# aouyang1/go-muse

Hardware: AMD Instinct MI355X
Metric: series-pairs XCorr/sec at N=4096, 1M-series batch; achieved HBM GB/s (higher is better)
Workload: dtype f64

## Files before the change

### go-muse_amd/csrc/foldk_device.h

```cpp
#pragma once
#include <hip/hip_runtime.h>
#include <stdint.h>

#include "fold_device.h"
#include "r16_device.h"

namespace muse {

namespace foldk {

using namespace occ4;
using namespace fold;

constexpr int XW = 544;

template <int PERM>
__device__ __forceinline__ constexpr int pr(int k)
{
    return PERM ? BR16(k) : k;
}

template <int MODE, int PERM, bool TAILBAR = false>
__device__ __forceinline__ void exchange_cross(double2 (&v)[16], double2 *xbuf, const int wave, const int t_, const int wcol = -1)
{
// ... 60 lines not shown
    const int rbase = 272 * hl + 17 * lo;
#pragma unroll
    for (int k = 0; k < 16; k++)
        lds_st2(xw + 17 * k + wbase, v[pr<PERM>(k)]);
    fence();
    asm volatile("" ::: "memory");
    fence();
#pragma unroll
    for (int e = 0; e < 16; e++)
        v[e] = lds_ld2(xw + rbase + e);
}

#if defined(__HIP_DEVICE_COMPILE__)
typedef __attribute__((address_space(3))) char *lds_ptr;
#define MUSE_LDS_ADDR(p) ((unsigned)(unsigned long long)(lds_ptr)(p))
#else
#define MUSE_LDS_ADDR(p) 0u
#endif
template <int PERM>
__device__ __forceinline__ void exchange_local(double2 (&v)[16], double2 *xw, const int t_)
{
    const int t = t_;
    const int hl = (t >> 4) & 3, lo = t & 15;
    const int wbase = 17 * hl + lo;
    const int rbase = 68 * (lo & 7) + 17 * hl;
#pragma unroll
    for (int k = 0; k < 8; k++)
        lds_st2(xw + 68 * k + wbase, v[pr<PERM>(k)]);
    const unsigned waddr = MUSE_LDS_ADDR(xw + wbase), raddr = MUSE_LDS_ADDR(xw + rbase);
    const unsigned long long first = __ballot(lo < 8);
    d2v w[16], d[8];
#pragma unroll
    for (int k = 0; k < 8; k++) {
        d[k].x = v[pr<PERM>(8 + k)].x;
        d[k].y = v[pr<PERM>(8 + k)].y;
    }
    unsigned long long sv;
    asm volatile("s_mov_b64 %[sv], exec\n\t"
                 "s_and_b64 exec, %[sv], %[m]\n\t"
                 "ds_read_b128 %[w0], %[ra]\n\t"
                 "ds_read_b128 %[w1], %[ra] offset:16\n\t"
                 "ds_read_b128 %[w2], %[ra] offset:32\n\t"
                 "ds_read_b128 %[w3], %[ra] offset:48\n\t"
                 "ds_read_b128 %[w4], %[ra] offset:64\n\t"
                 "ds_read_b128 %[w5], %[ra] offset:80\n\t"
                 "ds_read_b128 %[w6], %[ra] offset:96\n\t"
                 "ds_read_b128 %[w7], %[ra] offset:112\n\t"
                 "ds_read_b128 %[w8], %[ra] offset:128\n\t"
                 "ds_read_b128 %[w9], %[ra] offset:144\n\t"
                 "ds_read_b128 %[w10], %[ra] offset:160\n\t"
                 "ds_read_b128 %[w11], %[ra] offset:176\n\t"
                 "ds_read_b128 %[w12], %[ra] offset:192\n\t"
                 "ds_read_b128 %[w13], %[ra] offset:208\n\t"
                 "ds_read_b128 %[w14], %[ra] offset:224\n\t"
                 "ds_read_b128 %[w15], %[ra] offset:240\n\t"
                 "s_mov_b64 exec, %[sv]\n\t"
                 "ds_write_b128 %[wa], %[d0]\n\t"
                 "ds_write_b128 %[wa], %[d1] offset:1088\n\t"
                 "ds_write_b128 %[wa], %[d2] offset:2176\n\t"
                 "ds_write_b128 %[wa], %[d3] offset:3264\n\t"
                 "ds_write_b128 %[wa], %[d4] offset:4352\n\t"
                 "ds_write_b128 %[wa], %[d5] offset:5440\n\t"
                 "ds_write_b128 %[wa], %[d6] offset:6528\n\t"
                 "ds_write_b128 %[wa], %[d7] offset:7616\n\t"
                 "s_andn2_b64 exec, %[sv], %[m]\n\t"
                 "ds_read_b128 %[w0], %[ra]\n\t"
                 "ds_read_b128 %[w1], %[ra] offset:16\n\t"
                 "ds_read_b128 %[w2], %[ra] offset:32\n\t"
                 "ds_read_b128 %[w3], %[ra] offset:48\n\t"
                 "ds_read_b128 %[w4], %[ra] offset:64\n\t"
                 "ds_read_b128 %[w5], %[ra] offset:80\n\t"
                 "ds_read_b128 %[w6], %[ra] offset:96\n\t"
                 "ds_read_b128 %[w7], %[ra] offset:112\n\t"
                 "ds_read_b128 %[w8], %[ra] offset:128\n\t"
                 "ds_read_b128 %[w9], %[ra] offset:144\n\t"
                 "ds_read_b128 %[w10], %[ra] offset:160\n\t"
                 "ds_read_b128 %[w11], %[ra] offset:176\n\t"
                 "ds_read_b128 %[w12], %[ra] offset:192\n\t"
                 "ds_read_b128 %[w13], %[ra] offset:208\n\t"
                 "ds_read_b128 %[w14], %[ra] offset:224\n\t"
                 "ds_read_b128 %[w15], %[ra] offset:240\n\t"
                 "s_mov_b64 exec, %[sv]\n\t"
                 "s_waitcnt lgkmcnt(0)"
                 : [w0] "=&v"(w[0]), [w1] "=&v"(w[1]), [w2] "=&v"(w[2]), [w3] "=&v"(w[3]), [w4] "=&v"(w[4]),
                   [w5] "=&v"(w[5]), [w6] "=&v"(w[6]), [w7] "=&v"(w[7]), [w8] "=&v"(w[8]), [w9] "=&v"(w[9]),
                   [w10] "=&v"(w[10]), [w11] "=&v"(w[11]), [w12] "=&v"(w[12]), [w13] "=&v"(w[13]),
                   [w14] "=&v"(w[14]), [w15] "=&v"(w[15]), [sv] "=&s"(sv)
                 : [ra] "v"(raddr), [wa] "v"(waddr), [m] "s"(first), [d0] "v"(d[0]), [d1] "v"(d[1]), [d2] "v"(d[2]),
                   [d3] "v"(d[3]), [d4] "v"(d[4]), [d5] "v"(d[5]), [d6] "v"(d[6]), [d7] "v"(d[7])
                 : "memory", "scc");
#pragma unroll
    for (int e = 0; e < 16; e++)
        v[e] = make_double2(w[e].x, w[e].y);
}

struct G2Fetch {
    const double2 *p;
    int j;
    __device__ __forceinline__ double2 operator()(int s) const { return p[16 * s + j]; }
};
struct G3Fetch {
    const double2 *p;
    int t;
    __device__ __forceinline__ double2 operator()(int s) const
    {
        return ldg2(scalar_ptr_at(p, ((s + 1) & ~1) * 256), t - 256 * (s & 1));
    }
};

struct G3Derived {
    double2 g[8];
    __device__ __forceinline__ static double2 sq(const double2 w) { return make_double2(fma_(w.x, w.x, -(w.y * w.y)), (w.x + w.x) * w.y); }
    __device__ __forceinline__ static double2 mulc(const double2 w, const double c, const double s)
    {
        return make_double2(fma_(w.y, s, w.x * c), fma_(-w.x, s, w.y * c));
    }
    __device__ __forceinline__ G3Derived(const double2 *tab, int t)
    {
        constexpr double H = 0.70710678118654752440;
        const double2 w8 = G3Fetch{tab, t}(2), w16 = G3Fetch{tab, t}(4);
        g[2] = w8;
        g[4] = w16;
        g[1] = sq(w8);
        g[0] = sq(g[1]);
        g[3] = make_double2(H * (w8.x + w8.y), H * (w8.y - w8.x));
        g[5] = mulc(w16, C16_1, S16_1);
        g[6] = make_double2(H * (w16.x + w16.y), H * (w16.y - w16.x));
        g[7] = mulc(w16, S16_1, C16_1);
    }
    __device__ __forceinline__ double2 operator()(int s) const { return g[s]; }
};

template <typename F>
__device__ __forceinline__ void gdft16_nr_l2(double2 (&v)[16], F fetch)
{
    double2 ga[4], gb[4];
#pragma unroll
    for (int s = 0; s < 4; s++)
        ga[s] = fetch(s);
    gdft16_nr_s12(v, ga[0], ga[1]);
    fence();
#pragma unroll
    for (int s = 0; s < 4; s++)
        gb[s] = fetch(4 + s);
    fence();
    gdft16_nr_s3(v, ga[2], ga[3]);
    fence();
    fence();
    gdft16_nr_s4(v, gb[0], gb[1], gb[2], gb[3]);
}

constexpr int REC = 36;

__device__ __forceinline__ bool finalize(const double *r, const int series, const double invN, const double invNm1,
                                         double *mv_out, int *lag_out)
{
    double m[4], s[4], ix[4];
#pragma unroll
    for (int w = 0; w < 4; w++) {
        m[w] = r[6 * w + 3 * series];
        s[w] = r[6 * w + 3 * series + 1];
        ix[w] = r[6 * w + 3 * series + 2];
    }
    const double s2 = (r[24 + series] + r[26 + series]) + (r[28 + series] + r[30 + series]);
    const Stat st{r[32 + series], s2};
    double best = m[0], bsv = s[0], bidx = ix[0];
#pragma unroll
    for (int w = 1; w < 4; w++) {
        if (m[w] > best || (m[w] == best && ix[w] < bidx)) {
            best = m[w];
            bsv = s[w];
            bidx = ix[w];
        }
    }
    bool zero, nan;
    const double var = variance(st, invN, invNm1, zero, nan);
    const int idx = (best > 0.0) ? (int)bidx : 0;
    double y = __builtin_amdgcn_rsq(var);
    y = y * fma(-0.5 * var * y, y, 1.5);
    y = y * fma(-0.5 * var * y, y, 1.5);
    double mv = ((best > 0.0) ? bsv : s[0]) * y;
    int lag = idx > 2048 ? idx - 4096 : idx;
    if (zero) { mv = 0.0; lag = 0; }
    if (nan) { mv = __builtin_nan(""); lag = 0; }
    *mv_out = mv;
    *lag_out = lag;
    bool redo = nan;
    if (series == 0 && r[35] != 0.0) {
        const double s2b = (r[25] + r[27]) + (r[29] + r[31]);
        const Stat sb{r[33], s2b};
        bool zb, nb;
        const double varb = variance(sb, invN, invNm1, zb, nb);
        redo = redo || (!nb && sigma_spread_too_wide(var, varb));
    }
    return redo;
}

#define MUSE_HIWORD_CASE(m) case m: h = __builtin_amdgcn_readlane(__double2hiint(S == 0 ? v[BR16(m)].x : v[BR16(m)].y), l); break;
template <int S>
__device__ __forceinline__ int hiword_at(const double2 (&v)[16], const int m, const int l)
{
    int h = 0;
    switch (m) {
        MUSE_HIWORD_CASE(0) MUSE_HIWORD_CASE(1) MUSE_HIWORD_CASE(2) MUSE_HIWORD_CASE(3)
        MUSE_HIWORD_CASE(4) MUSE_HIWORD_CASE(5) MUSE_HIWORD_CASE(6) MUSE_HIWORD_CASE(7)
        MUSE_HIWORD_CASE(8) MUSE_HIWORD_CASE(9) MUSE_HIWORD_CASE(10) MUSE_HIWORD_CASE(11)
        MUSE_HIWORD_CASE(12) MUSE_HIWORD_CASE(13) MUSE_HIWORD_CASE(14) MUSE_HIWORD_CASE(15)
    }
    return h;
}
#undef MUSE_HIWORD_CASE
__device__ __forceinline__ void lowest_hit(const unsigned acc, int &m_out, int &l_out)
{
    unsigned long long c = __ballot(acc != 0u);
    int bm = 16, bl = 0;
    while (c != 0ull) {
        const int l = __ffsll((long long)c) - 1;
        const int m = __ffs((int)__builtin_amdgcn_readlane((int)acc, l)) - 1;
        if (m < bm) {
            bm = m;
            bl = l;
        }
        c &= c - 1ull;
    }
    m_out = bm;
    l_out = bl;
}
__device__ __forceinline__ void wave_argmax_store(const double2 (&v)[16], const int wave, const int lane, double *ra_)
{
    double ma = 0.0, mb = 0.0;
#pragma unroll
    for (int k = 0; k < 16; k++) {
        ma = fmax(ma, fabs(v[k].x));
        mb = fmax(mb, fabs(v[k].y));
    }
    const double wa = wave_max_nonneg(ma), wb = wave_max_nonneg(mb);
    unsigned accA = 0u, accB = 0u;
#pragma unroll
    for (int m = 15; m >= 0; m--) {
        const int k = BR16(m);
        asm("v_cmp_eq_f64 vcc, |%1|, %2\n\tv_addc_co_u32 %0, vcc, %0, %0, vcc" : "+v"(accA) : "v"(v[k].x), "s"(wa) : "vcc");
        asm("v_cmp_eq_f64 vcc, |%1|, %2\n\tv_addc_co_u32 %0, vcc, %0, %0, vcc" : "+v"(accB) : "v"(v[k].y), "s"(wb) : "vcc");
    }
    int widxA = 0x7fffffff, widxB = 0x7fffffff;
    double svA = 0.0, svB = 0.0;
    if (__double_as_longlong(wa) != 0ll) {
        int m, l;
        lowest_hit(accA, m, l);
        if (m < 16) {
            widxA = wave * 64 + l + 256 * m;
            svA = (hiword_at<0>(v, m, l) < 0) ? -wa : wa;
        }
    }
    if (__double_as_longlong(wb) != 0ll) {
        int m, l;
        lowest_hit(accB, m, l);
        if (m < 16) {
            widxB = wave * 64 + l + 256 * m;
            svB = (hiword_at<1>(v, m, l) < 0) ? -wb : wb;
        }
    }
    const double cc0a = v[0].x, cc0b = v[0].y;
    if (lane == 0) {
        ra_[0] = widxA == 0x7fffffff ? 0.0 : wa;
        ra_[1] = widxA == 0x7fffffff ? cc0a : svA;
        ra_[2] = (double)widxA;
        ra_[3] = widxB == 0x7fffffff ? 0.0 : wb;
        ra_[4] = widxB == 0x7fffffff ? cc0b : svB;
        ra_[5] = (double)widxB;
    }
}

template <int S>
__device__ __forceinline__ void wave_argmax_store_one(const double2 (&v)[16], const int wave, const int lane, double *out3)
{
    double ma = 0.0;
#pragma unroll
    for (int k = 0; k < 16; k++)
        ma = fmax(ma, fabs(S == 0 ? v[k].x : v[k].y));
    const double wa = wave_max_nonneg(ma);
    unsigned acc = 0u;
#pragma unroll
    for (int m = 15; m >= 0; m--) {
        const int k = BR16(m);
        asm("v_cmp_eq_f64 vcc, |%1|, %2\n\tv_addc_co_u32 %0, vcc, %0, %0, vcc" : "+v"(acc) : "v"(S == 0 ? v[k].x : v[k].y), "s"(wa) : "vcc");
    }
    int widx = 0x7fffffff;
    double sv = 0.0;
    if (__double_as_longlong(wa) != 0ll) {
        int m, l;
        lowest_hit(acc, m, l);
        if (m < 16) {
            widx = wave * 64 + l + 256 * m;
            sv = (hiword_at<S>(v, m, l) < 0) ? -wa : wa;
        }
    }
    const double cc0 = S == 0 ? v[0].x : v[0].y;
    if (lane == 0) {
        out3[0] = widx == 0x7fffffff ? 0.0 : wa;
        out3[1] = widx == 0x7fffffff ? cc0 : sv;
        out3[2] = (double)widx;
    }
}

__device__ __forceinline__ void xc_stage1_pre(double2 (&v)[16], const double2 (&xf)[16])
{
#pragma unroll
    for (int i = 0; i < 4; i++) {
        bf_xc(v[BR16(2 * i)], v[BR16(2 * i) + 1], xf[2 * i], xf[2 * i + 8]);
        bf_xc(v[BR16(2 * i + 1)], v[BR16(2 * i + 1) + 1], xf[2 * i + 1], xf[2 * i + 9]);
    }
}

template <typename F>
__device__ __forceinline__ void xc_stage1(double2 (&v)[16], F xcl)
{
    double2 xa[4], xb[4];
#define MUSE_XC_LOAD(dst, i)          \
    dst[0] = xcl(2 * (i));            \
    dst[1] = xcl(2 * (i) + 8);        \
    dst[2] = xcl(2 * (i) + 1);        \
    dst[3] = xcl(2 * (i) + 9);
#define MUSE_XC_USE(src, i)                                                      \
    bf_xc(v[BR16(2 * (i))], v[BR16(2 * (i)) + 1], src[0], src[1]);               \
    bf_xc(v[BR16(2 * (i) + 1)], v[BR16(2 * (i) + 1) + 1], src[2], src[3]);
    MUSE_XC_LOAD(xa, 0)
    MUSE_XC_LOAD(xb, 1)
    fence();
    MUSE_XC_USE(xa, 0)
    fence();
    MUSE_XC_LOAD(xa, 2)
    MUSE_XC_USE(xb, 1)
    fence();
    MUSE_XC_LOAD(xb, 3)
    MUSE_XC_USE(xa, 2)
    fence();
    MUSE_XC_USE(xb, 3)
#undef MUSE_XC_LOAD
#undef MUSE_XC_USE
}

}

}
```

### go-muse_amd/csrc/n4096_pair_device.h

```cpp
#pragma once
#include "foldk_device.h"

namespace muse {

namespace foldk {

#if defined(__HIP_DEVICE_COMPILE__)
typedef d2v __attribute__((address_space(1))) *zc_out_ptr;
typedef double __attribute__((address_space(1))) *zstat_out_ptr;
typedef const double __attribute__((address_space(4))) *zstat_in_ptr;
#endif

struct PairThread {
    int t, lane, wave;
    double invN, invNm1;
};
template <bool PADDED>
__device__ __forceinline__ PairThread pair_prologue(const FusedParams &p, double2 *g2s, double *prev_row, const int rec_stride)
{
    PairThread th;
    th.t = threadIdx.x;
    th.lane = th.t & 63;
    th.wave = __builtin_amdgcn_readfirstlane(th.t >> 6);
    th.invN = PADDED ? p.invN : 1.0 / 4096.0;
    th.invNm1 = PADDED ? p.invNm1 : 1.0 / 4095.0;
    if (th.t < 128)
        g2s[th.t] = p.g2[th.t];
    if (th.t < 2)
        prev_row[rec_stride * th.t] = -1.0;
    return th;
}

template <bool PIN>
__device__ __forceinline__ int tl(const int t)
{
    int x = t;
    if (PIN)
        asm volatile("" : "+v"(x));
    return x;
}

template <typename T>
__device__ __forceinline__ gptr<T> lane_entry(const T *tab, const long long off, const int j, const int t)
{
    return scalar_ptr_at(tab, off + 256 * ((j + 1) & ~1)) + (t - 256 * (j & 1));
}
struct XcFetch {
    const double2 *xcp;
    int t;
    __device__ __forceinline__ double2 operator()(int j) const { return ldg2(lane_entry(xcp, 0, j, t), 0); }
};

template <bool PADDED, bool F32, bool SLIDE = false>
__device__ __forceinline__ void request_rows(RawPair &raw, const FusedParams &p, const long long pr, const int t, const int pad)
{
    constexpr bool WIDE = !PADDED && !F32;
    if (SLIDE && WIDE)
        issue_row_loads_wide_slide(raw, p, pr, t);
    else if (SLIDE && F32)
        issue_row_loads_slide<PADDED>(raw, p.rows32, p, pr, t, pad);
    else if (SLIDE)
        issue_row_loads_slide<PADDED>(raw, p.rows, p, pr, t, pad);
    else if (WIDE)
        issue_row_loads_wide(raw, p, pr, t);
    else
        issue_row_loads<PADDED, F32>(raw, p, pr, t, pad);
}

#define MUSE_CONSUME_ROWS(WIDE, raw, v, part, t, lane, wave, rA, hasB)      \
    {                                                                       \
        const double KA = (raw).ka, KB = (raw).kb;                          \
        double qa = 0.0, qb = 0.0;                                          \
        if (WIDE)                                                           \
            widen_rows(raw);                                                \
        _Pragma("unroll") for (int i = 0; i < 16; i++) {                    \
            const double da = (raw).a[i] - KA, db = (raw).b[i] - KB;        \
            (v)[i] = make_double2(da, db);                                  \
            qa = fma(da, da, qa);                                           \
            qb = fma(db, db, qb);                                           \
        }                                                                   \
        qa = wave_sum_dpp(qa);                                              \
        qb = wave_sum_dpp(qb);                                              \
        if ((lane) == 0) {                                                  \
            (part)[2 * (wave)] = qa;                                        \
            (part)[2 * (wave) + 1] = qb;                                    \
        }                                                                   \
        if ((t) == 0) {                                                     \
            (part)[10] = (double)(rA);                                      \
            (part)[11] = (hasB) ? 1.0 : 0.0;                                \
        }                                                                   \
    }

template <bool PADDED>
__device__ __forceinline__ void take_dc(double2 (&v)[16], const int t, double &s1a, double &s1b)
{
    s1a = readlane_f64(v[0].x, 0);
    s1b = readlane_f64(v[0].y, 0);
    if (!PADDED) {
        v[0].x = (t == 0) ? 0.0 : v[0].x;
        v[0].y = (t == 0) ? 0.0 : v[0].y;
    }
}

__device__ __forceinline__ void finalize_pair(const double *prec, const int series, const bool writer, const double invN,
                                              const double invNm1, const FusedParams &p)
{
    if (writer && series < 2 && prec[34] >= 0.0 && (series == 0 || prec[35] != 0.0)) {
        const long long row = (long long)prec[34] + series;
        if (finalize(prec, series, invN, invNm1, p.mv + row, p.lag + row)) {
            const int slot = atomicAdd(p.ovf_count, 1);
            p.ovf_list[slot] = row >> 1;
        }
    }
}

struct Nothing {
    __device__ __forceinline__ void operator()() const {}
};
template <int B, typename Between = Nothing>
__device__ __forceinline__ void correct_padded(double2 (&v)[16], const double *c1, const int t, const double mA, const double mB,
                                               Between between = Between())
{
#pragma unroll
    for (int h = 0; h < 16 / B; h++) {
        double cq[B];
#pragma unroll
        for (int k = 0; k < B; k++)
            cq[k] = *lane_entry(c1, 0, B * h + k, t);
        fence();
        between();
#pragma unroll
        for (int k = 0; k < B; k++) {
            const int r = BR16(B * h + k);
            v[r] = make_double2(fma(-mA, cq[k], v[r].x), fma(-mB, cq[k], v[r].y));
        }
    }
}

__device__ __forceinline__ void request_z(d2v (&zn)[16], const SpectrumCacheArgs &c, const long long pr, const int t)
{
#pragma unroll
    for (int i = 0; i < 16; i++)
        zn[i] = __builtin_nontemporal_load((gptr<d2v>)lane_entry(c.zc, (pr - c.pair0) * 4096, i, t));
}
__device__ __forceinline__ void load_pair_stats(double (&st)[10], const double *zstat, const long long rel)
{
#if defined(__HIP_DEVICE_COMPILE__)
    const zstat_in_ptr sp = (zstat_in_ptr)(unsigned long long)(zstat + rel * ZC_STAT);
#pragma unroll
    for (int k = 0; k < 10; k++)
        st[k] = sp[k];
#endif
}
__device__ __forceinline__ void publish_pair_stats(double *rec, const double (&st)[10], const int t, const long long rA, const bool hasB)
{
    if (t == 0) {
#pragma unroll
        for (int k = 0; k < 10; k++)
            rec[24 + k] = st[k];
        rec[34] = (double)rA;
        rec[35] = hasB ? 1.0 : 0.0;
    }
}

struct NoTap {
    static constexpr long long first = 0;
    __device__ __forceinline__ void operator()(const double2 (&)[16], const double *, double, double, long long, int) const {}
};

template <bool TIMING, bool PADDED, bool F32, bool WIN, bool SLIDE, typename Tap>
__device__ __forceinline__ void pair_loop_from_rows(const FusedParams &p, const Tap tap)
{
    __shared__ double2 xbuf[OCC_XBUF];
    __shared__ double2 g2s[128];
    __shared__ double red[2 * REC];
    __shared__ int next_s[2];
    const PairThread th = pair_prologue<PADDED>(p, g2s, red + 34, REC);
    const int t = th.t, lane = th.lane, wave = th.wave;
    const double invN = th.invN, invNm1 = th.invNm1;
    double2 *const xw = xbuf + XW * wave;
    const int pad = PADDED ? 4096 - p.N : 0;
    __syncthreads();
    PhaseClock<TIMING> clk;
    clk.start();

    int parity = 0;
    const long long first = tap.first, total = first + p.npairs;
    RawPair raw;
    constexpr bool WIDE = !PADDED && !F32;
    request_rows<PADDED, F32, SLIDE>(raw, p, first + blockIdx.x < total ? first + (long long)blockIdx.x : first, t, pad);

    long long nextpair = 0;
    for (long long pair = first + blockIdx.x; pair < total; pair = nextpair) {
        const long long rA = 2 * pair;
        const bool hasB = rA + 1 < p.M;
        double *const rec = red + REC * parity;
        const double *const prec = red + REC * (parity ^ 1);
        if (t == 0)
            next_s[parity] = (int)gridDim.x + atomicAdd(p.work_counter, 1);
        if (SLIDE) {
            fence();
            asm volatile("s_waitcnt vmcnt(0) lgkmcnt(0)\n\ts_barrier" ::: "memory");
            fence();
            if (WIDE)
                store_slid_rows_wide(raw, p, pair, t);
            else if (F32)
                store_slid_rows<PADDED>(raw, const_cast<float *>(p.rows32), p, pair, t, pad);
            else
                store_slid_rows<PADDED>(raw, const_cast<double *>(p.rows), p, pair, t, pad);
        }
        double2 v[16];
        if (TIMING)
            asm volatile("s_waitcnt vmcnt(0)" ::: "memory");
        clk.template stamp<0>();
        MUSE_CONSUME_ROWS(WIDE, raw, v, rec + 24, t, lane, wave, rA, hasB)
        clk.template stamp<1>();
        dft16_nr(v);
        clk.template stamp<2>();
        exchange_cross<0, 1, true>(v, xbuf, wave, t, WIDE ? wide_column(t) : -1);
        finalize_pair(prec, wave, lane == 0, invN, invNm1, p);
        clk.template stamp<3>();
        gdft16_nr(v, G2Fetch{g2s, t >> 4});
        clk.template stamp<4>();
        exchange_local<1>(v, xw, tl<PADDED>(t));
        clk.template stamp<5>();
        gdft16_nr_l2(v, G3Derived(p.g3a, t));
        double s1a, s1b;
        take_dc<PADDED>(v, t, s1a, s1b);
        tap(v, rec, s1a, s1b, pair - first, t);
        clk.template stamp<6>();
        xc_stage1(v, XcFetch{p.xcp, t});
        dft16_rn_s234(v);
        clk.template stamp<7>();
        exchange_local<0>(v, xw, tl<PADDED>(t));
        if (PADDED && wave == 0 && lane == 0) {
            rec[32] = s1a;
            rec[33] = s1b;
        }
        clk.template stamp<8>();
        gdft16_nr(v, G2Fetch{g2s, t & 15});
        clk.template stamp<9>();
        exchange_cross<1, 1>(v, xbuf, wave, t);
        clk.template stamp<10>();
        nextpair = first + __builtin_amdgcn_readfirstlane(next_s[parity]);
        long long nxt = nextpair;
        nxt = nxt < total ? nxt : first;
        gdft16_nr_l2(v, G3Derived(p.g3b, t));
        if (PADDED)
            correct_padded<8>(v, p.c1, t, rec[32] * invN, rec[33] * invN);
        if (WIN)
            mask_window<true, 256>(v, tl<PADDED>(t), p.win_lpos, 4096 - p.win_lneg);
        clk.template stamp<11>();
        if (F32) {
            fence();
            request_rows<PADDED, F32, SLIDE>(raw, p, nxt, t, pad);
            fence();
        }
        wave_argmax_store(v, wave, lane, rec + 6 * wave);
        clk.template stamp<13>();
        fence();
        if (!F32)
            request_rows<PADDED, F32, SLIDE>(raw, p, nxt, t, pad);
        fence();
        if (wave == 0 && lane == 0) {
            rec[32] = s1a;
            rec[33] = s1b;
        }
        parity ^= 1;
        clk.template stamp<12>();
    }
    lds_barrier();
    finalize_pair(red + REC * (parity ^ 1), t, true, invN, invNm1, p);
    if (TIMING && p.dbg && lane == 0) {
#pragma unroll
        for (int i = 0; i < NPHASE; i++)
            p.dbg[((long long)blockIdx.x * 4 + wave) * NPHASE + i] = clk.acc[i];
    }
}

}

}
```

### go-muse_amd/csrc/xcorr_kernels.h

```cpp
#pragma once
#include <hip/hip_runtime.h>
#include <stdint.h>
#include <type_traits>

#include "muse_hip.h"

namespace muse {

enum { KERNEL_GENERIC = 0, KERNEL_R16_OCC3 = 6, KERNEL_STOCKHAM = 10, KERNEL_R16_FOLD = 11, KERNEL_SMALL = 12, KERNEL_LONG = 13, KERNEL_REAL = 14, KERNEL_REAL_SPLIT = 15 };

struct FusedParams {
    const double *rows;
    const float *rows32;
    long long M;
    long long stride;
    long long npairs;
    int N;
    int n;
    int logn;
    int normalize_y;
    const double2 *xc;
    const double2 *tw1;
    const double2 *tw2;
    const double2 *xcp;
    const double2 *g2;
    const double2 *g3a;
    const double2 *g3b;
    const double2 *gsmall;
    const double2 *gsmall_b;
    const double2 *wsplit;
    const double2 *xcw;
    const double2 *twl;
    const double *c1;
    int R;
    const double2 *const *xcp_many;
    double *const *mv_many;
    int *const *lag_many;
    const double *const *c1_many;
    const float2 *const *xcf_many;
    unsigned *const *flags_many;
    double *const *var_many;
    double2 *zscratch;
    int zslots;
    const double2 *twm;
    double2 *gscratch;
    double *mv;
    int *lag;
    double *cc_out;
    int *nil_out;
    unsigned long long *dbg;
    const float2 *twmf;
    const float2 *tw1f;
    const float2 *tw2f;
    const float2 *xcf;
    const double *xs;
    double screen_delta;
    unsigned *scr_flags;
    double *scr_var;
    int scr_max_lag;
    int scr_need_sign;
    int *ovf_count;
    int *work_counter;
    long long *ovf_list;
    const long long *pair_list;
    const int *pair_count;
    long long dense_total;
    long long gscratch_slices;
    const double *xrows;
    long long xstride;
    int Nx;
    double invN, invNm1;
    int win, win_lpos, win_lneg;
    const void *slide_tails;
    int slide_k;
};
inline FusedParams with_reciprocals(FusedParams p)
{
    p.invN = 1.0 / (double)p.N;
    p.invNm1 = 1.0 / (double)(p.N - 1);
    return p;
}
inline bool window_bounds_ok(const FusedParams &p)
{
    return !p.win || (p.win_lpos >= 0 && p.win_lneg >= 0 && p.win_lpos <= 2048 && p.win_lneg <= 2047);
}
template <typename F>
inline void with_bools(F f)
{
    f();
}
template <typename F, typename... Rest>
inline void with_bools(F f, bool b, Rest... rest)
{
    if (b)
        with_bools([&](auto... flags) { f(std::true_type{}, flags...); }, rest...);
    else
        with_bools([&](auto... flags) { f(std::false_type{}, flags...); }, rest...);
}

hipError_t launch_fused(const FusedParams &p, int variant, int num_cus, hipStream_t stream);
hipError_t launch_fused_occ4(const FusedParams &p, int num_cus, hipStream_t stream);
hipError_t launch_screen_pass(const FusedParams &p, int num_cus, hipStream_t stream);
hipError_t launch_screen_pass_many(const FusedParams &p, int num_cus, hipStream_t stream);
hipError_t launch_screen_pass_stk(const FusedParams &p, int num_cus, hipStream_t stream);
enum : unsigned { SCR_IN = 1u, SCR_OUT = 2u, SCR_POS = 4u, SCR_NEG = 8u, SCR_REFINE = 16u, SCR_NAN = 32u };
hipError_t launch_fused_fold(const FusedParams &p, int num_cus, hipStream_t stream);
hipError_t launch_fused_multi(const FusedParams &p, int num_cus, hipStream_t stream);
constexpr int ZC_STAT = 16;
constexpr long long ZC_PAIR_BYTES = 4096 * 16 + ZC_STAT * 8;
struct SpectrumCacheArgs {
    double2 *zc;
    double *zstat;
    long long pair0;
    long long zpairs;
};
hipError_t launch_cache_fill(const FusedParams &p, const SpectrumCacheArgs &c, int num_cus, hipStream_t stream);
hipError_t launch_cached(const FusedParams &p, const SpectrumCacheArgs &c, int num_cus, hipStream_t stream, bool occ4 = false);
hipError_t launch_fused_small(const FusedParams &p, int num_cus, hipStream_t stream);
hipError_t launch_fused_stockham(const FusedParams &p, int num_cus, hipStream_t stream);
hipError_t launch_fused_long(const FusedParams &p, int num_cus, hipStream_t stream);
hipError_t launch_real_split_tables(const double2 *xc, double2 *out, hipStream_t stream);
hipError_t launch_real8k_tables(const double2 *xc, double2 *out, hipStream_t stream);
hipError_t launch_two_sided_real(const FusedParams &p, int num_cus, hipStream_t stream);
hipError_t launch_fused_real_split(const FusedParams &p, int num_cus, hipStream_t stream);
hipError_t launch_fused_real(const FusedParams &p, int num_cus, hipStream_t stream);
hipError_t launch_two_sided(const FusedParams &p, int num_cus, hipStream_t stream);
hipError_t launch_two_sided_small(const FusedParams &p, int num_cus, hipStream_t stream);
hipError_t launch_lane_order_rows(const double2 *in, double2 *out, int R1, hipStream_t stream);
hipError_t launch_lane_order(const double2 *in, double2 *out, hipStream_t stream);
hipError_t launch_indicator_corr(const double *xs, int n, int pad, double *c1, hipStream_t stream);
hipError_t launch_ref_spectrum(const double *ref_dev, int N, int n, int logn, int normalize, double x_scale,
                               double xc_scale, const double2 *twm, double2 *X, double2 *xc, float2 *xcf, double *xs,
                               double2 *gscratch, int *status, hipStream_t stream);
constexpr int SMALL_MAX_N = 16384;
constexpr int GENERIC_LDS_MAX_N = 8192;
constexpr int GENERIC_MAX_N = 65536;
constexpr int GENERIC_GLOBAL_WGS_PER_CU = 2;
constexpr int STOCKHAM_GLOBAL_WGS_PER_CU = 2;
constexpr int LONG_WGS_PER_CU = 4;
constexpr int GSCRATCH_SLICES_PER_CU = 4;
static_assert(LONG_WGS_PER_CU <= GSCRATCH_SLICES_PER_CU && GENERIC_GLOBAL_WGS_PER_CU <= GSCRATCH_SLICES_PER_CU &&
                  2 * STOCKHAM_GLOBAL_WGS_PER_CU <= GSCRATCH_SLICES_PER_CU,
              "the scratch buffer is sized for GSCRATCH_SLICES_PER_CU slices per CU");
constexpr int WIN_KC = 1024;
constexpr int WIN_E_TAIL = 128;
static_assert(2 * MUSE_LAG_WINDOW_MAX + 2 <= WIN_E_TAIL, "the staged image covers every lag of the widest window");
struct WindowShape {
    const double *rows;
    long long M, stride;
    int N;
    int L, Lneg;
    double invN, invNm1;
    int origin;
};
struct WindowParams : WindowShape {
    const double *e;
    const double *pw;
    double *mv;
    int *lag;
};
inline bool window_wide(const double *rows, long long stride) { return stride % 2 == 0 && ((uintptr_t)rows & 15) == 0; }
inline long long window_e_len(int N) { return (long long)((N + WIN_KC - 1) / WIN_KC) * WIN_KC + WIN_E_TAIL; }
hipError_t launch_window_tables(const double *xs, int N, int n, int origin, int W, double *e, long long e_len, double *pw, hipStream_t stream);
hipError_t launch_window(const WindowParams &p, hipStream_t stream);
void slide_score_plan(int N, int k, bool wide, int *load_bytes, int *store_bytes);
hipError_t launch_window_slide(const WindowParams &p, const double *tails, int k, hipStream_t stream);
constexpr int WIN_ROWS_FULL_SPLIT = 16;
constexpr int WIN_ROWS_MIN_CHUNKS = 2;
constexpr bool WIN_ROWS_SPLIT_ENABLED = true;
int window_rows_plan(long long M, int N, int num_cus, int *chunks_per_slice);
long long window_split_slab_doubles(const WindowShape &p);
hipError_t launch_window_split(const WindowParams &p, int S, double *slabs, hipStream_t stream);
constexpr int WIN_PANEL_ROWS = 128;
constexpr int WIN_PANEL_MAX_ROWS = 2048;
static_assert(WIN_PANEL_MAX_ROWS == MUSE_RUN_ROWS_LAG_RANGE_MAX && WIN_PANEL_ROWS + 2 <= WIN_E_TAIL + 2, "a panel's image is a chunk's");
int window_panels(int W);
long long window_panels_e_len(int N, int W);
hipError_t launch_window_tables_wide(const double *xs, int N, int n, int origin, int W, double *e, long long e_len, double *pw, hipStream_t stream);
constexpr int WIN_PANEL_BALANCE = 10;
int window_panels_plan(long long M, int N, int num_cus, int W, int *panels);
long long window_panels_slab_doubles();
hipError_t launch_window_panels(const WindowParams &p, int S, double *slabs, hipStream_t stream);
constexpr int WINM_MAX_TILES = 8;
constexpr int WINM_PACK_MAX_ROWS = 48;
constexpr int WINM_IMG_DOUBLES = 4608;
struct WindowManyParams : WindowShape {
    int R;
    const double *const *e;
    const double *const *pw;
    double *const *mv;
    int *const *lag;
    int kc, img, buf, parts;
};
int window_many_img(int W, int kc);
int window_many_max_refs(int W);
int window_many_kc(int W, int refs);
int window_many_plan(int R, int W, int *launch_of, int *tiles_of);
hipError_t launch_window_many(WindowManyParams p, hipStream_t stream);
hipError_t launch_direct(const double *x, int lenx, const double *y, int leny, int n, int normalize_x,
                         int normalize_y, double x_scale, double cc_scale, double *cc, int *lag, double *mv,
                         int *status, hipStream_t stream);
hipError_t launch_two_sided_rescue(const double *xrows, long long xstride, int Nx, const double *yrows, long long ystride, int Ny,
                                   int n, int normalize, const long long *list, int count, int *code, double2 *scale,
                                   hipStream_t stream);
hipError_t launch_scale_listed_rows(const double *src, long long stride, int N, const long long *list, const double2 *g, int which,
                                    int count, double *dst, hipStream_t stream);
hipError_t launch_synth(double *rows, long long stride, long long first, long long count, long long global_first,
                        int N, unsigned long long seed, unsigned flags, hipStream_t stream);
hipError_t launch_synth_f32(float *rows, long long stride, long long first, long long count, long long global_first,
                            int N, unsigned long long seed, unsigned flags, hipStream_t stream);
hipError_t launch_synth_ref(double *ref, int N, unsigned long long seed, hipStream_t stream);
hipError_t launch_row_gather(const void *src, bool src_f32, void *dst, bool dst_f32, const long long *idx, long long count,
                             int N, int num_cus, bool nontemporal, hipStream_t stream);
int slide_unit_bytes(int N, int k, bool f32);
hipError_t launch_row_slide(void *rows, bool f32, long long count, int N, int k, const void *tails, int num_cus,
                            hipStream_t stream);

hipError_t launch_clock_probe(unsigned long long *out, int *count, int max_windows, double window_ms, double total_ms,
                              hipStream_t stream);
hipError_t launch_wave_argmax_probe(const double *ccA, const double *ccB, double *out24, hipStream_t stream);

constexpr int TOPN_CHUNK = 4096;
constexpr int TOPN_DEVICE_MAX = 256;
constexpr int EXACT_FEED_MAX_GROUPS = 65536;

struct GroupWork {
    unsigned long long *key;
    long long *first;
    long long *win;
};

struct SelectParams {
    const double *mv;
    const int *lag;
    long long M;
    const int *group_id;
    int G;
    int abs_scores;
    int max_lag;
    double threshold;
    int sign_filter;
    long long series_offset;
    const unsigned char *include;
    int partial;
};

struct ScreenSelect {
    const double *mv;
    const double *var;
    const unsigned *flags;
    long long M;
    double threshold;
    int sign_filter;
    int abs_scores;
    double E;
    const int *group_id;
    int G;
};
struct ScreenGroupWork {
    long long *first;
    unsigned long long *glo, *gmay, *gkplus;
// ... 45 lines not shown
```

### go-muse_amd/csrc/xcorr_r16_cached.hip

```cpp
#include <hip/hip_runtime.h>
#include <stdint.h>
#include <algorithm>

#include "n4096_pair_device.h"

namespace muse {

struct CacheTap {
    const SpectrumCacheArgs c;
    const long long first;
    __device__ __forceinline__ void operator()(const double2 (&v)[16], const double *rec, const double s1a, const double s1b,
                                               const long long rel, const int t) const
    {
#if defined(__HIP_DEVICE_COMPILE__)
        if (rel < c.zpairs) {
            const foldk::zc_out_ptr zo = (foldk::zc_out_ptr)(unsigned long long)(c.zc + rel * 4096) + t;
#pragma unroll
            for (int i = 0; i < 16; i++)
                __builtin_nontemporal_store(occ4::d2v{v[i].x, v[i].y}, zo + 256 * i);
            if (t < 10) {
                const foldk::zstat_out_ptr so = (foldk::zstat_out_ptr)(unsigned long long)(c.zstat + rel * ZC_STAT);
                so[t] = t < 8 ? rec[24 + t] : (t == 8 ? s1a : s1b);
            }
        }
#endif
    }
};

template <bool PADDED>
__global__ __launch_bounds__(OCC_THREADS, 4) void xcorr_cache_fill_n4096(const FusedParams p, const SpectrumCacheArgs c)
{
    foldk::pair_loop_from_rows<false, PADDED, false, false, false>(p, CacheTap{c, c.pair0});
}

struct G3Lazy {
    double2 w8, w16;
    __device__ __forceinline__ double2 operator()(int s) const
    {
        constexpr double H = 0.70710678118654752440;
        switch (s) {
        case 0: return foldk::G3Derived::sq(foldk::G3Derived::sq(w8));
        case 1: return foldk::G3Derived::sq(w8);
        case 2: return w8;
        case 3: return make_double2(H * (w8.x + w8.y), H * (w8.y - w8.x));
        case 4: return w16;
        case 5: return foldk::G3Derived::mulc(w16, fold::C16_1, fold::S16_1);
        case 6: return make_double2(H * (w16.x + w16.y), H * (w16.y - w16.x));
        default: return foldk::G3Derived::mulc(w16, fold::S16_1, fold::C16_1);
        }
    }
};

constexpr int ZC_CLAIM = 2;

template <bool PADDED>
__global__ __launch_bounds__(OCC_THREADS, 2) void xcorr_cached_n4096(const FusedParams p, const SpectrumCacheArgs c)
{
    using namespace occ4;
    using namespace fold;
    using namespace foldk;
    __shared__ double2 xbuf[OCC_XBUF_FULL];
    __shared__ double2 g2s[128];
    __shared__ double red[2 * REC];
    __shared__ int next_s[2];
    const PairThread th = pair_prologue<PADDED>(p, g2s, red + 34, REC);
    const int t = th.t, lane = th.lane, wave = th.wave;
    const double invN = th.invN, invNm1 = th.invNm1;
    double2 *const xw = xbuf + 1088 * wave;
    const long long first = c.pair0, total = c.pair0 + p.npairs;
    constexpr bool AHEAD = !PADDED;
    constexpr int ch = ZC_CLAIM;

    if (t == 0)
        next_s[1] = (int)gridDim.x + atomicAdd(p.work_counter, 1);
    d2v zn[16];
    request_z(zn, c, first + (long long)ch * blockIdx.x, t);
    double2 xf[16];
#pragma unroll
    for (int j = 0; j < 16; j++)
        xf[j] = XcFetch{p.xcp, t}(j);
    G3Lazy g3{G3Fetch{p.g3b, t}(2), G3Fetch{p.g3b, t}(4)};
    __syncthreads();

    int parity = 0, cpar = 0;
    long long pair = first + (long long)ch * blockIdx.x;
    long long cbeg = pair, cend = pair + ch < total ? pair + ch : total;
    long long nchunk = first + (long long)ch * __builtin_amdgcn_readfirstlane(next_s[1]), after = 0;
    while (pair < total) {
        const bool claiming = pair == cbeg;
        const long long nextpair = pair + 1 < cend ? pair + 1 : nchunk;
        const long long rA = 2 * pair;
        const bool hasB = rA + 1 < p.M;
        double *const rec = red + REC * parity;
        const double *const prec = red + REC * (parity ^ 1);
        double st[10];
        load_pair_stats(st, c.zstat, pair - first);
        double2 v[16];
#pragma unroll
        for (int i = 0; i < 16; i++)
            v[i] = make_double2(zn[i].x, zn[i].y);
        xc_stage1_pre(v, xf);
        int claim = 0;
#pragma unroll
        for (int i = 0; i < 16; i += 4)
            asm volatile("" : "+v"(v[i].x), "+v"(v[i].y), "+v"(v[i + 1].x), "+v"(v[i + 1].y), "+v"(v[i + 2].x), "+v"(v[i + 2].y), "+v"(v[i + 3].x), "+v"(v[i + 3].y));
#if defined(__HIP_DEVICE_COMPILE__)
        if (claiming && t == 0) {
            unsigned long long wc = (unsigned long long)p.work_counter;
            asm volatile("" : "+v"(wc));
            claim = __hip_atomic_fetch_add((int __attribute__((address_space(1))) *)wc, 1, __ATOMIC_RELAXED, __HIP_MEMORY_SCOPE_AGENT);
        }
#endif
        const long long nxt = nextpair < total ? nextpair : first;
        if (AHEAD) {
            fence();
            request_z(zn, c, nxt, t);
            fence();
        }
        asm volatile("" : "+v"(g3.w8.x), "+v"(g3.w8.y), "+v"(g3.w16.x), "+v"(g3.w16.y));
        dft16_rn_s234(v);
        exchange_local_full<0>(v, xw, t);
        gdft16_nr(v, G2Fetch{g2s, t & 15});
        if (claiming && t == 0)
            next_s[cpar] = (int)gridDim.x + claim;
        exchange_cross_full<1, 1>(v, xbuf, t);
        lds_barrier();
        finalize_pair(prec, wave, lane == 0, invN, invNm1, p);
        publish_pair_stats(rec, st, t, rA, hasB);
        if (claiming) {
            after = first + (long long)ch * __builtin_amdgcn_readfirstlane(next_s[cpar]);
            cpar ^= 1;
        }
        gdft16_nr_l2(v, g3);
        if (PADDED)
            correct_padded<16>(v, p.c1, t, st[8] * invN, st[9] * invN, [&]() __attribute__((always_inline)) {
                request_z(zn, c, nxt, t);
                fence();
            });
        wave_argmax_store(v, wave, lane, rec + 6 * wave);
        parity ^= 1;
        if (pair + 1 < cend) {
            pair++;
        } else {
            pair = cbeg = nchunk;
            cend = pair + ch < total ? pair + ch : total;
            nchunk = after;
        }
    }
    lds_barrier();
    finalize_pair(red + REC * (parity ^ 1), t, true, invN, invNm1, p);
}

template <bool PADDED>
__global__ __launch_bounds__(OCC_THREADS, 4) void xcorr_cached_n4096_occ4(const FusedParams p, const SpectrumCacheArgs c)
{
    using namespace occ4;
    using namespace fold;
    using namespace foldk;
    __shared__ double2 xbuf[OCC_XBUF];
    __shared__ double2 g2s[128];
    __shared__ double red[2 * REC];
    __shared__ int next_s[2];
    const PairThread th = pair_prologue<PADDED>(p, g2s, red + 34, REC);
    const int t = th.t, lane = th.lane, wave = th.wave;
    const double invN = th.invN, invNm1 = th.invNm1;
    double2 *const xw = xbuf + XW * wave;
    __syncthreads();

    int parity = 0;
    const long long first = c.pair0, total = c.pair0 + p.npairs;
    d2v zn[16];
    request_z(zn, c, first + blockIdx.x < total ? first + (long long)blockIdx.x : first, t);

    long long nextpair = 0;
    for (long long pair = first + blockIdx.x; pair < total; pair = nextpair) {
        const long long rA = 2 * pair;
        const bool hasB = rA + 1 < p.M;
        double *const rec = red + REC * parity;
        const double *const prec = red + REC * (parity ^ 1);
        if (t == 0)
            next_s[parity] = (int)gridDim.x + atomicAdd(p.work_counter, 1);
        double st[10];
        load_pair_stats(st, c.zstat, pair - first);
        double2 v[16];
#pragma unroll
        for (int i = 0; i < 16; i++)
            v[i] = make_double2(zn[i].x, zn[i].y);
        xc_stage1(v, XcFetch{p.xcp, t});
        dft16_rn_s234(v);
        exchange_local<0>(v, xw, tl<PADDED>(t));
        gdft16_nr(v, G2Fetch{g2s, t & 15});
        exchange_cross<1, 1, true>(v, xbuf, wave, t);
        finalize_pair(prec, wave, lane == 0, invN, invNm1, p);
        publish_pair_stats(rec, st, t, rA, hasB);
        nextpair = first + __builtin_amdgcn_readfirstlane(next_s[parity]);
        long long nxt = nextpair;
        nxt = nxt < total ? nxt : first;
        gdft16_nr_l2(v, G3Derived(p.g3b, t));
        if (PADDED)
            correct_padded<8>(v, p.c1, t, st[8] * invN, st[9] * invN);
        wave_argmax_store(v, wave, lane, rec + 6 * wave);
        fence();
        request_z(zn, c, nxt, t);
        fence();
        parity ^= 1;
    }
    lds_barrier();
    finalize_pair(red + REC * (parity ^ 1), t, true, invN, invNm1, p);
}

static bool cache_launch_ok(const FusedParams &p, const SpectrumCacheArgs &c)
{
    return p.rows && !p.rows32 && p.n == 4096 && p.N > 2048 && p.N <= 4096 && p.npairs > 0 && c.pair0 >= 0 &&
           2 * (c.pair0 + p.npairs) <= p.M + 1 && p.work_counter && p.ovf_count && p.ovf_list && p.g2 && p.g3a && p.g3b && p.xcp &&
           (p.N == 4096 || p.c1);
}

hipError_t launch_cache_fill(const FusedParams &p_in, const SpectrumCacheArgs &c, int num_cus, hipStream_t stream)
{
    const FusedParams p = with_reciprocals(p_in);
    if (!cache_launch_ok(p, c) || c.zpairs < 0 || c.zpairs > p.npairs || (c.zpairs > 0 && (!c.zc || !c.zstat)) ||
        2 * (c.pair0 + c.zpairs) > p.M)
        return hipErrorInvalidValue;
    const dim3 g((unsigned)std::min<long long>(p.npairs, (long long)num_cus * 4)), b(OCC_THREADS);
    with_bools([&](auto padded) { hipLaunchKernelGGL((xcorr_cache_fill_n4096<decltype(padded)::value>), g, b, 0, stream, p, c); }, p.N < 4096);
    return hipGetLastError();
}

hipError_t launch_cached(const FusedParams &p_in, const SpectrumCacheArgs &c, int num_cus, hipStream_t stream, bool occ4)
{
    const FusedParams p = with_reciprocals(p_in);
    if (!cache_launch_ok(p, c) || !c.zc || !c.zstat || c.zpairs < p.npairs || 2 * (c.pair0 + p.npairs) > p.M)
        return hipErrorInvalidValue;
    const dim3 g((unsigned)(occ4 ? std::min<long long>(p.npairs, (long long)num_cus * 4)
                                 : std::min<long long>((p.npairs + ZC_CLAIM - 1) / ZC_CLAIM, (long long)num_cus * 2))), b(OCC_THREADS);
    with_bools([&](auto four, auto padded) {
        if (decltype(four)::value)
            hipLaunchKernelGGL((xcorr_cached_n4096_occ4<decltype(padded)::value>), g, b, 0, stream, p, c);
        else
            hipLaunchKernelGGL((xcorr_cached_n4096<decltype(padded)::value>), g, b, 0, stream, p, c);
    }, occ4, p.N < 4096);
    return hipGetLastError();
}

}

#undef MUSE_CONSUME_ROWS
```

Baseline: 164.3 million.

## Precompute per-pair finalize verdicts in cache fill and prefetch them in cached kernels

The cache-fill pass now stores each series' inverse sigma and a bitmask of zero/NaN/spread verdicts next to the cached spectrum stats. The cached kernels skip recomputing variance, rsq refinement and spread checks, and simply combine the wave argmax records with the stored y and flags. The stats load is now prefetched one iteration ahead with an explicit waitcnt, and LDS record publication shrinks to a vector store. This adds stats-layout coupling between the fill and read kernels, and limits M to 32-bit rows.

```diff
diff --git a/go-muse_amd/csrc/foldk_device.h b/go-muse_amd/csrc/foldk_device.h
--- a/go-muse_amd/csrc/foldk_device.h
+++ b/go-muse_amd/csrc/foldk_device.h
@@ -236,47 +236,77 @@
 
 constexpr int REC = 36;
 
-__device__ __forceinline__ bool finalize(const double *r, const int series, const double invN, const double invNm1,
-                                         double *mv_out, int *lag_out)
-{
-    double m[4], s[4], ix[4];
-#pragma unroll
-    for (int w = 0; w < 4; w++) {
-        m[w] = r[6 * w + 3 * series];
-        s[w] = r[6 * w + 3 * series + 1];
-        ix[w] = r[6 * w + 3 * series + 2];
-    }
+constexpr unsigned VERDICT_ZERO_A = 1u, VERDICT_NAN_A = 2u, VERDICT_SPREAD = 4u, VERDICT_ZERO_B = 8u, VERDICT_NAN_B = 16u;
+__device__ __forceinline__ unsigned verdict_zero(const int series) { return series == 0 ? VERDICT_ZERO_A : VERDICT_ZERO_B; }
+__device__ __forceinline__ unsigned verdict_nan(const int series) { return series == 0 ? VERDICT_NAN_A : VERDICT_NAN_B; }
+__device__ __forceinline__ unsigned verdict_redo(const int series) { return series == 0 ? VERDICT_NAN_A | VERDICT_SPREAD : VERDICT_NAN_B; }
+
+__device__ __forceinline__ double record_variance(const double *r, const int series, const double invN, const double invNm1, bool &zero, bool &nan)
+{
     const double s2 = (r[24 + series] + r[26 + series]) + (r[28 + series] + r[30 + series]);
     const Stat st{r[32 + series], s2};
-    double best = m[0], bsv = s[0], bidx = ix[0];
-#pragma unroll
-    for (int w = 1; w < 4; w++) {
-        if (m[w] > best || (m[w] == best && ix[w] < bidx)) {
-            best = m[w];
-            bsv = s[w];
-            bidx = ix[w];
-        }
-    }
-    bool zero, nan;
-    const double var = variance(st, invN, invNm1, zero, nan);
-    const int idx = (best > 0.0) ? (int)bidx : 0;
+    return variance(st, invN, invNm1, zero, nan);
+}
+__device__ __forceinline__ double inv_sigma(const double var)
+{
     double y = __builtin_amdgcn_rsq(var);
     y = y * fma(-0.5 * var * y, y, 1.5);
     y = y * fma(-0.5 * var * y, y, 1.5);
-    double mv = ((best > 0.0) ? bsv : s[0]) * y;
+    return y;
+}
+struct WaveRecords {
+    double m[4], s[4], ix[4];
+};
+__device__ __forceinline__ WaveRecords load_wave_records(const double *r, const int series)
+{
+    WaveRecords w;
+#pragma unroll
+    for (int k = 0; k < 4; k++) {
+        w.m[k] = r[6 * k + 3 * series];
+        w.s[k] = r[6 * k + 3 * series + 1];
+        w.ix[k] = r[6 * k + 3 * series + 2];
+    }
+    return w;
+}
+__device__ __forceinline__ void combine(const WaveRecords &w, const double y, const bool zero, const bool nan, double *mv_out, int *lag_out)
+{
+    double best = w.m[0], bsv = w.s[0], bidx = w.ix[0];
+#pragma unroll
+    for (int k = 1; k < 4; k++) {
+        if (w.m[k] > best || (w.m[k] == best && w.ix[k] < bidx)) {
+            best = w.m[k];
+            bsv = w.s[k];
+            bidx = w.ix[k];
+        }
+    }
+    const int idx = (best > 0.0) ? (int)bidx : 0;
+    double mv = ((best > 0.0) ? bsv : w.s[0]) * y;
     int lag = idx > 2048 ? idx - 4096 : idx;
     if (zero) { mv = 0.0; lag = 0; }
     if (nan) { mv = __builtin_nan(""); lag = 0; }
     *mv_out = mv;
     *lag_out = lag;
+}
+
+template <typename Keep>
+__device__ __forceinline__ bool finalize(const double *r, const int series, const double invN, const double invNm1,
+                                         double *mv_out, int *lag_out, const Keep keep)
+{
+    const WaveRecords w = load_wave_records(r, series);
+    bool zero, nan;
+    const double var = record_variance(r, series, invN, invNm1, zero, nan);
+    const double y = inv_sigma(var);
+    combine(w, y, zero, nan, mv_out, lag_out);
     bool redo = nan;
+    unsigned bits = (zero ? verdict_zero(series) : 0u) | (nan ? verdict_nan(series) : 0u);
     if (series == 0 && r[35] != 0.0) {
-        const double s2b = (r[25] + r[27]) + (r[29] + r[31]);
-        const Stat sb{r[33], s2b};
         bool zb, nb;
-        const double varb = variance(sb, invN, invNm1, zb, nb);
-        redo = redo || (!nb && sigma_spread_too_wide(var, varb));
-    }
+        const double varb = record_variance(r, 1, invN, invNm1, zb, nb);
+        const bool spread = !nb && sigma_spread_too_wide(var, varb);
+        redo = redo || spread;
+        bits |= (zb ? VERDICT_ZERO_B : 0u) | (nb ? VERDICT_NAN_B : 0u) | (spread ? VERDICT_SPREAD : 0u);
+    }
+    keep(y, bits);
     return redo;
 }
 
diff --git a/go-muse_amd/csrc/n4096_pair_device.h b/go-muse_amd/csrc/n4096_pair_device.h
--- a/go-muse_amd/csrc/n4096_pair_device.h
+++ b/go-muse_amd/csrc/n4096_pair_device.h
@@ -102,12 +102,14 @@
     }
 }
 
+template <typename Tap>
 __device__ __forceinline__ void finalize_pair(const double *prec, const int series, const bool writer, const double invN,
-                                              const double invNm1, const FusedParams &p)
+                                              const double invNm1, const FusedParams &p, const Tap &tap)
 {
     if (writer && series < 2 && prec[34] >= 0.0 && (series == 0 || prec[35] != 0.0)) {
         const long long row = (long long)prec[34] + series;
-        if (finalize(prec, series, invN, invNm1, p.mv + row, p.lag + row)) {
+        if (finalize(prec, series, invN, invNm1, p.mv + row, p.lag + row,
+                     [&](const double y, const unsigned bits) __attribute__((always_inline)) { tap.verdict(row >> 1, series, y, bits); })) {
             const int slot = atomicAdd(p.ovf_count, 1);
             p.ovf_list[slot] = row >> 1;
         }
@@ -143,29 +145,72 @@
     for (int i = 0; i < 16; i++)
         zn[i] = __builtin_nontemporal_load((gptr<d2v>)lane_entry(c.zc, (pr - c.pair0) * 4096, i, t));
 }
-__device__ __forceinline__ void load_pair_stats(double (&st)[10], const double *zstat, const long long rel)
-{
+struct PairVerdict {
+    double yA, yB, s1a, s1b;
+    unsigned bits;
+};
+template <bool SUMS, bool IN_LOOP>
+__device__ __forceinline__ PairVerdict load_pair_verdict(const double *zstat, const long long rel_)
+{
+    PairVerdict q = {};
 #if defined(__HIP_DEVICE_COMPILE__)
+    long long rel = rel_;
+    if (IN_LOOP) {
+        fence();
+        __builtin_amdgcn_s_waitcnt(0xc07f);
+        asm volatile("" : "+s"(rel));
+    }
     const zstat_in_ptr sp = (zstat_in_ptr)(unsigned long long)(zstat + rel * ZC_STAT);
-#pragma unroll
-    for (int k = 0; k < 10; k++)
-        st[k] = sp[k];
+    if (SUMS) {
+        q.s1a = sp[8];
+        q.s1b = sp[9];
+    }
+    q.yA = sp[ZC_VERDICT];
+    q.yB = sp[ZC_VERDICT + 1];
+    q.bits = ((const unsigned __attribute__((address_space(4))) *)sp)[2 * (ZC_VERDICT + 2)];
+    if (IN_LOOP)
+        fence();
 #endif
-}
-__device__ __forceinline__ void publish_pair_stats(double *rec, const double (&st)[10], const int t, const long long rA, const bool hasB)
+    return q;
+}
+struct ReaderHead {
+    unsigned bits;
+    int row, hasB, unused;
+};
+__device__ __forceinline__ void reader_prologue(double *red, const int t)
+{
+    if (t < 2)
+        *(ReaderHead *)(red + REC * t + 26) = ReaderHead{0u, -1, 0, 0};
+}
+__device__ __forceinline__ void publish_pair_verdict(double *rec, const PairVerdict &q, const int t, const long long rA, const bool hasB)
 {
     if (t == 0) {
-#pragma unroll
-        for (int k = 0; k < 10; k++)
-            rec[24 + k] = st[k];
-        rec[34] = (double)rA;
-        rec[35] = hasB ? 1.0 : 0.0;
+        *(double2 *)(rec + 24) = make_double2(q.yA, q.yB);
+        *(ReaderHead *)(rec + 26) = ReaderHead{q.bits, (int)rA, hasB ? 1 : 0, 0};
+    }
+}
+__device__ __forceinline__ void finalize_pair_cached(const double *prec, const int series, const bool writer, const FusedParams &p)
+{
+    if (writer && series < 2) {
+        const WaveRecords w = load_wave_records(prec, series);
+        const double y = prec[24 + series];
+        const ReaderHead h = *(const ReaderHead *)(prec + 26);
+        fence();
+        if (h.row >= 0 && (series == 0 || h.hasB != 0)) {
+            const long long row = (long long)h.row + series;
+            combine(w, y, (h.bits & verdict_zero(series)) != 0u, (h.bits & verdict_nan(series)) != 0u, p.mv + row, p.lag + row);
+            if (h.bits & verdict_redo(series)) {
+                const int slot = atomicAdd(p.ovf_count, 1);
+                p.ovf_list[slot] = row >> 1;
+            }
+        }
     }
 }
 
 struct NoTap {
     static constexpr long long first = 0;
     __device__ __forceinline__ void operator()(const double2 (&)[16], const double *, double, double, long long, int) const {}
+    __device__ __forceinline__ void verdict(long long, int, double, unsigned) const {}
 };
 
 template <bool TIMING, bool PADDED, bool F32, bool WIN, bool SLIDE, typename Tap>
@@ -218,7 +263,7 @@
         dft16_nr(v);
         clk.template stamp<2>();
         exchange_cross<0, 1, true>(v, xbuf, wave, t, WIDE ? wide_column(t) : -1);
-        finalize_pair(prec, wave, lane == 0, invN, invNm1, p);
+        finalize_pair(prec, wave, lane == 0, invN, invNm1, p, tap);
         clk.template stamp<3>();
         gdft16_nr(v, G2Fetch{g2s, t >> 4});
         clk.template stamp<4>();
@@ -270,7 +315,7 @@
         clk.template stamp<12>();
     }
     lds_barrier();
-    finalize_pair(red + REC * (parity ^ 1), t, true, invN, invNm1, p);
+    finalize_pair(red + REC * (parity ^ 1), t, true, invN, invNm1, p, tap);
     if (TIMING && p.dbg && lane == 0) {
 #pragma unroll
         for (int i = 0; i < NPHASE; i++)
diff --git a/go-muse_amd/csrc/xcorr_kernels.h b/go-muse_amd/csrc/xcorr_kernels.h
--- a/go-muse_amd/csrc/xcorr_kernels.h
+++ b/go-muse_amd/csrc/xcorr_kernels.h
@@ -107,6 +107,7 @@
 hipError_t launch_fused_fold(const FusedParams &p, int num_cus, hipStream_t stream);
 hipError_t launch_fused_multi(const FusedParams &p, int num_cus, hipStream_t stream);
 constexpr int ZC_STAT = 16;
+constexpr int ZC_VERDICT = 10;
 constexpr long long ZC_PAIR_BYTES = 4096 * 16 + ZC_STAT * 8;
 struct SpectrumCacheArgs {
     double2 *zc;
diff --git a/go-muse_amd/csrc/xcorr_r16_cached.hip b/go-muse_amd/csrc/xcorr_r16_cached.hip
--- a/go-muse_amd/csrc/xcorr_r16_cached.hip
+++ b/go-muse_amd/csrc/xcorr_r16_cached.hip
@@ -22,6 +22,18 @@
                 const foldk::zstat_out_ptr so = (foldk::zstat_out_ptr)(unsigned long long)(c.zstat + rel * ZC_STAT);
                 so[t] = t < 8 ? rec[24 + t] : (t == 8 ? s1a : s1b);
             }
+        }
+#endif
+    }
+    __device__ __forceinline__ void verdict(const long long pair, const int series, const double y, const unsigned bits) const
+    {
+#if defined(__HIP_DEVICE_COMPILE__)
+        const long long rel = pair - first;
+        if (rel < c.zpairs) {
+            const foldk::zstat_out_ptr so = (foldk::zstat_out_ptr)(unsigned long long)(c.zstat + rel * ZC_STAT);
+            so[ZC_VERDICT + series] = y;
+            if (series == 0)
+                so[ZC_VERDICT + 2] = __hiloint2double(0, (int)bits);
         }
 #endif
     }
@@ -61,11 +73,12 @@
     using namespace foldk;
     __shared__ double2 xbuf[OCC_XBUF_FULL];
     __shared__ double2 g2s[128];
-    __shared__ double red[2 * REC];
+    __shared__ alignas(16) double red[2 * REC];
     __shared__ int next_s[2];
     const PairThread th = pair_prologue<PADDED>(p, g2s, red + 34, REC);
     const int t = th.t, lane = th.lane, wave = th.wave;
-    const double invN = th.invN, invNm1 = th.invNm1;
+    const double invN = th.invN;
+    reader_prologue(red, t);
     double2 *const xw = xbuf + 1088 * wave;
     const long long first = c.pair0, total = c.pair0 + p.npairs;
     constexpr bool AHEAD = !PADDED;
@@ -75,6 +88,7 @@
         next_s[1] = (int)gridDim.x + atomicAdd(p.work_counter, 1);
     d2v zn[16];
     request_z(zn, c, first + (long long)ch * blockIdx.x, t);
+    PairVerdict qn = load_pair_verdict<PADDED, false>(c.zstat, (long long)ch * blockIdx.x);
     double2 xf[16];
 #pragma unroll
     for (int j = 0; j < 16; j++)
@@ -93,8 +107,7 @@
         const bool hasB = rA + 1 < p.M;
         double *const rec = red + REC * parity;
         const double *const prec = red + REC * (parity ^ 1);
-        double st[10];
-        load_pair_stats(st, c.zstat, pair - first);
+        const PairVerdict q = qn;
         double2 v[16];
 #pragma unroll
         for (int i = 0; i < 16; i++)
@@ -125,15 +138,16 @@
             next_s[cpar] = (int)gridDim.x + claim;
         exchange_cross_full<1, 1>(v, xbuf, t);
         lds_barrier();
-        finalize_pair(prec, wave, lane == 0, invN, invNm1, p);
-        publish_pair_stats(rec, st, t, rA, hasB);
+        finalize_pair_cached(prec, wave, lane == 0, p);
+        publish_pair_verdict(rec, q, t, rA, hasB);
         if (claiming) {
             after = first + (long long)ch * __builtin_amdgcn_readfirstlane(next_s[cpar]);
             cpar ^= 1;
         }
+        qn = load_pair_verdict<PADDED, true>(c.zstat, nxt - first);
         gdft16_nr_l2(v, g3);
         if (PADDED)
-            correct_padded<16>(v, p.c1, t, st[8] * invN, st[9] * invN, [&]() __attribute__((always_inline)) {
+            correct_padded<16>(v, p.c1, t, q.s1a * invN, q.s1b * invN, [&]() __attribute__((always_inline)) {
                 request_z(zn, c, nxt, t);
                 fence();
             });
@@ -148,7 +162,7 @@
         }
     }
     lds_barrier();
-    finalize_pair(red + REC * (parity ^ 1), t, true, invN, invNm1, p);
+    finalize_pair_cached(red + REC * (parity ^ 1), t, true, p);
 }
 
 template <bool PADDED>
@@ -159,11 +173,12 @@
     using namespace foldk;
     __shared__ double2 xbuf[OCC_XBUF];
     __shared__ double2 g2s[128];
-    __shared__ double red[2 * REC];
+    __shared__ alignas(16) double red[2 * REC];
     __shared__ int next_s[2];
     const PairThread th = pair_prologue<PADDED>(p, g2s, red + 34, REC);
     const int t = th.t, lane = th.lane, wave = th.wave;
-    const double invN = th.invN, invNm1 = th.invNm1;
+    const double invN = th.invN;
+    reader_prologue(red, t);
     double2 *const xw = xbuf + XW * wave;
     __syncthreads();
 
@@ -171,6 +186,7 @@
     const long long first = c.pair0, total = c.pair0 + p.npairs;
     d2v zn[16];
     request_z(zn, c, first + blockIdx.x < total ? first + (long long)blockIdx.x : first, t);
+    PairVerdict qn = load_pair_verdict<PADDED, false>(c.zstat, first + blockIdx.x < total ? (long long)blockIdx.x : 0);
 
     long long nextpair = 0;
     for (long long pair = first + blockIdx.x; pair < total; pair = nextpair) {
@@ -180,8 +196,7 @@
         const double *const prec = red + REC * (parity ^ 1);
         if (t == 0)
             next_s[parity] = (int)gridDim.x + atomicAdd(p.work_counter, 1);
-        double st[10];
-        load_pair_stats(st, c.zstat, pair - first);
+        const PairVerdict q = qn;
         double2 v[16];
 #pragma unroll
         for (int i = 0; i < 16; i++)
@@ -191,14 +206,15 @@
         exchange_local<0>(v, xw, tl<PADDED>(t));
         gdft16_nr(v, G2Fetch{g2s, t & 15});
         exchange_cross<1, 1, true>(v, xbuf, wave, t);
-        finalize_pair(prec, wave, lane == 0, invN, invNm1, p);
-        publish_pair_stats(rec, st, t, rA, hasB);
+        finalize_pair_cached(prec, wave, lane == 0, p);
+        publish_pair_verdict(rec, q, t, rA, hasB);
         nextpair = first + __builtin_amdgcn_readfirstlane(next_s[parity]);
         long long nxt = nextpair;
         nxt = nxt < total ? nxt : first;
+        qn = load_pair_verdict<PADDED, true>(c.zstat, nxt - first);
         gdft16_nr_l2(v, G3Derived(p.g3b, t));
         if (PADDED)
-            correct_padded<8>(v, p.c1, t, st[8] * invN, st[9] * invN);
+            correct_padded<8>(v, p.c1, t, q.s1a * invN, q.s1b * invN);
         wave_argmax_store(v, wave, lane, rec + 6 * wave);
         fence();
         request_z(zn, c, nxt, t);
@@ -206,7 +222,7 @@
         parity ^= 1;
     }
     lds_barrier();
-    finalize_pair(red + REC * (parity ^ 1), t, true, invN, invNm1, p);
+    finalize_pair_cached(red + REC * (parity ^ 1), t, true, p);
 }
 
 static bool cache_launch_ok(const FusedParams &p, const SpectrumCacheArgs &c)
@@ -230,7 +246,8 @@
 hipError_t launch_cached(const FusedParams &p_in, const SpectrumCacheArgs &c, int num_cus, hipStream_t stream, bool occ4)
 {
     const FusedParams p = with_reciprocals(p_in);
-    if (!cache_launch_ok(p, c) || !c.zc || !c.zstat || c.zpairs < p.npairs || 2 * (c.pair0 + p.npairs) > p.M)
+    if (!cache_launch_ok(p, c) || !c.zc || !c.zstat || c.zpairs < p.npairs || 2 * (c.pair0 + p.npairs) > p.M ||
+        p.M > 0x7fffffffLL)
         return hipErrorInvalidValue;
     const dim3 g((unsigned)(occ4 ? std::min<long long>(p.npairs, (long long)num_cus * 4)
                                  : std::min<long long>((p.npairs + ZC_CLAIM - 1) / ZC_CLAIM, (long long)num_cus * 2))), b(OCC_THREADS);
```

Result: faster. 168.8 million (median of 6 runs) (+2.8%).
